# tjake/Jlama

Hardware: NVIDIA B200
Metric: decode tokens/s (higher is better)
Workload: dtype int8xint4->f32

## Files before the change

include/jlama_b200.h:

```cpp
#ifndef JLAMA_B200_H
#define JLAMA_B200_H

#include <stdint.h>

#ifdef __cplusplus
extern "C" {
#endif

#define JL_OK 0
#define JL_ERR_INVALID (-1)
#define JL_ERR_CUDA (-2)
#define JL_ERR_OOM (-3)
#define JL_ERR_UNSUPPORTED (-4)
#define JL_ERR_NCCL (-5)

#define JL_F32 0
#define JL_BF16 1
#define JL_Q4 2
#define JL_I8 3

typedef struct jl_ctx jl_ctx;
typedef struct jl_model jl_model;

int jl_init(int device, jl_ctx **out, int64_t *info );
int jl_shutdown(jl_ctx *ctx);
const char *jl_last_error(jl_ctx *ctx);
const char *jl_version(void);
int jl_sync(jl_ctx *ctx);
int64_t jl_kernel_launches(jl_ctx *ctx);

int jl_debug_ktrace(jl_ctx *ctx, int capacity);
int jl_debug_ktrace_clear(jl_ctx *ctx);
int jl_debug_ktrace_read(jl_ctx *ctx, uint64_t *out, int max_slots);
int jl_debug_gemv_bench(jl_ctx *ctx, int64_t b_id, int n, int m, int mode, int iters, int use_pdl, double *avg_us);

int jl_debug_gemm_tc_bench(jl_ctx *ctx, int64_t b_id, int t, int iters, double *avg_us);

int64_t jl_register_tensor(jl_ctx *ctx, int dtype, int64_t rows, int64_t cols, const void *data, const float *scales);
int jl_unregister_tensor(jl_ctx *ctx, int64_t id);

int jl_gemm(jl_ctx *ctx, int a_dtype, const void *a, const float *a_scales, int a_col_off, int lda, int64_t b_id,
            int b_col_off, float *r, int roffset, int m, int n0, int n, int k, int ldc);
int jl_gemm_batch(jl_ctx *ctx, int batch_num, int a_dtype, const void *a, const float *a_scales, int a_col_off, int lda,
                  const int64_t *b_ids, int b_col_off, float *const *r, int roffset, int m, int n0, int n, int k,
                  int ldc);
int jl_gemm_tc(jl_ctx *ctx, int a_dtype, const void *a, int a_col_off, int lda, int64_t b_id, int b_col_off, float *r,
               int roffset, int m, int n0, int n, int k, int ldc);
int jl_gemm_host(jl_ctx *ctx, int a_dtype, const void *a, int a_col_off, int lda, int b_dtype, const void *b,
                 int b_col_off, int ldb, float *r, int roffset, int m, int n0, int n, int k, int ldc);

int jl_accumulate(jl_ctx *ctx, float *a, int a_rows, int lda, int b_dtype, const void *b, const float *b_scales,
                  int b_rows, int ldb, int offset, int length);
int jl_maccumulate(jl_ctx *ctx, float *a, int a_rows, int lda, const float *b, int b_rows, int ldb, int offset,
                   int length);
int jl_scale(jl_ctx *ctx, float factor, float *x, int rows, int ldx, int offset, int length);
int jl_saxpy(jl_ctx *ctx, float alpha, const float *x, float *y, int xoffset, int yoffset, int limit);
int jl_saxpy_batch(jl_ctx *ctx, const float *alpha, const float *x, int ldx, float *y, int xoffset, int yoffset,
                   int limit, int a_offset, int x_row_offset, int batch);
int jl_quantize_q8(jl_ctx *ctx, const float *x, int rows, int ldx, int offset, int length, int8_t *q, float *scales);
int jl_quantize_bf16(jl_ctx *ctx, const float *x, int rows, int ldx, int offset, int length, uint16_t *out);
int jl_quantize_q4_weights(jl_ctx *ctx, const float *x, int64_t rows, int64_t cols, uint8_t *q, float *scales);
int jl_quantize_q8_weights(jl_ctx *ctx, const float *x, int64_t rows, int64_t cols, int8_t *q, float *scales);

int jl_rmsnorm(jl_ctx *ctx, const float *x, int rows, int ldx, int w_dtype, const void *w, float weight_adjustment,
               float eps, int embedding_length, int offset, int length, float *out);
int jl_layernorm(jl_ctx *ctx, const float *x, int rows, int ldx, int w_dtype, const void *w, int b_dtype, const void *bias, float eps,
                 int embedding_length, int offset, int length, float *out);
#define JL_ACT_SILU 0
#define JL_ACT_GELU 1
// ... 180 lines not shown
```

jlama_b200/csrc/jl_model.cu:

```cuda
#include "jl_common.cuh"
#include <string>
#include "jl_pdecode.cuh"

#include <chrono>
#include <map>
#include <math.h>
#include <new>
#include <stdio.h>
#include <stdlib.h>
#include <string.h>

int jl_comm_allreduce_dev(jl_ctx *ctx, cudaStream_t stream, float *buf, size_t count);
int jl_comm_allgather_dev(jl_ctx *ctx, cudaStream_t stream, const void *send, void *recv, size_t bytes_per_rank);

struct jl_model {
    jl_ctx *ctx = nullptr;
    std::recursive_mutex mu;
    jl_model_config cfg;
    jl_dctx d;
    cudaStream_t stream = nullptr;
    bool finalized = false;
    DevTensor g[3];
    bool g_set[3] = {false, false, false};
    std::vector<DevTensor> l;
// ... 14 lines not shown
    int max_splits = 32;
    int32_t *d_tokens = nullptr, *d_positions = nullptr, *d_sessions = nullptr, *d_next = nullptr, *d_hist = nullptr,
            *d_counter = nullptr;
    void *argmax_scratch = nullptr;
    int32_t *h_pinned = nullptr;
    int hist_cap = 0;
    std::map<long long, cudaGraphExec_t> graphs;
    std::map<long long, long long> graph_launches;
    std::vector<cudaEvent_t> ev_pool;
    size_t ev_used = 0;
    cudaEvent_t ev_begin = nullptr, ev_end = nullptr;
    double last_total_ms = 0, last_gemv_ms = 0;
    bool timing_valid = false;
    int64_t weight_bytes = 0;
    unsigned *fda_done = nullptr;
    std::vector<DevTensor> aux;
    std::vector<char> aux_set;
    DevTensor gaux[2];
    bool gaux_set[2] = {false, false};
    int n_exp = 0, exp_k = 0;
    std::vector<DevTensor> moe_gate;
    std::vector<DevTensor> moe_w;
    std::vector<char> moe_set;
    void **moe_wtab = nullptr;
    float **moe_stab = nullptr;
    float *moe_logits = nullptr;
    int32_t *moe_sel = nullptr;
    bool pd_ok = false;
    int pd_wdtype = JL_Q4;
    std::vector<PdLayer> pd_layers;
    unsigned long long *pd_sync = nullptr, *pd_slots = nullptr, *pd_trace = nullptr;
    unsigned *pd_att_done = nullptr;
    int pd_vocab0 = 0, pd_vocab_rows = 0;
    uint4 *ll_o = nullptr, *ll_d = nullptr, *ll_a = nullptr;
    struct KvSpill {
        std::vector<std::pair<int, int>> pages;
        std::vector<char> bytes;
    };
    std::map<int64_t, KvSpill> spills;
    int64_t next_spill = 1;
    uint4 *peer_ll_o[PD_MAX_TP] = {}, *peer_ll_d[PD_MAX_TP] = {}, *peer_ll_a[PD_MAX_TP] = {};
    float *peer_logits[PD_MAX_TP] = {};
    std::vector<void *> ipc_opened;
};

#define M_CHECK(expr)                 \
    do {                              \
        int _rc = (expr);             \
        if (_rc != JL_OK) return _rc; \
    } while (0)

static bool use_pdl(const jl_model *m) {
    static int env = -1;
    if (env < 0) {
        const char *e = getenv("JL_PDL");
        env = e ? (atoi(e) ? 1 : 0) : 2;
    }
    if (m->cfg.flags & JL_MODEL_NO_PDL) return false;
    if (env != 2) return env == 1;
    return (m->cfg.flags & JL_MODEL_PDL) != 0;
}
static bool use_graph(const jl_model *m) { return !(m->cfg.flags & JL_MODEL_NO_GRAPH); }
static bool use_pd(const jl_model *m) {
    static int env = -1;
    if (env < 0) {
        const char *e = getenv("JL_PERSISTENT");
// ... 380 lines not shown
                JL_CUDA_CHECK(ctx, cudaMemset(m->ll_d, 0, lines * 16));
                JL_CUDA_CHECK(ctx, cudaMemset(m->ll_a, 0, (size_t)PD_MAX_TP * 16));
                void *local[4] = {m->ll_o, m->ll_d, m->ll_a, m->logits};
                cudaIpcMemHandle_t mine[4];
                for (int i = 0; i < 4; i++) JL_CUDA_CHECK(ctx, cudaIpcGetMemHandle(&mine[i], local[i]));
                cudaIpcMemHandle_t *d_send = nullptr, *d_recv = nullptr;
                M_CHECK(dev_alloc(ctx, (void **)&d_send, sizeof mine));
                M_CHECK(dev_alloc(ctx, (void **)&d_recv, sizeof mine * W));
                JL_CUDA_CHECK(ctx, cudaMemcpy(d_send, mine, sizeof mine, cudaMemcpyHostToDevice));
                int rc = jl_comm_allgather_dev(ctx, m->stream, d_send, d_recv, sizeof mine);
                if (rc == JL_OK && cudaStreamSynchronize(m->stream) != cudaSuccess) rc = jl_set_error(ctx, JL_ERR_CUDA, "handle exchange failed");
                std::vector<cudaIpcMemHandle_t> all((size_t)4 * W);
                if (rc == JL_OK) JL_CUDA_CHECK(ctx, cudaMemcpy(all.data(), d_recv, sizeof mine * W, cudaMemcpyDeviceToHost));
                cudaFree(d_send);
                cudaFree(d_recv);
                if (rc != JL_OK) return rc;
                for (int r = 0; r < W; r++) {
                    void *ptrs[4];
                    for (int i = 0; i < 4; i++) {
                        if (r == c.tp_rank) {
                            ptrs[i] = local[i];
                        } else {
                            cudaError_t e = cudaIpcOpenMemHandle(&ptrs[i], all[(size_t)r * 4 + i], cudaIpcMemLazyEnablePeerAccess);
                            if (e != cudaSuccess)
                                return jl_set_error(ctx, JL_ERR_CUDA, "cudaIpcOpenMemHandle(rank %d): %s (peer access over NVLink is required)", r,
                                                    cudaGetErrorString(e));
                            m->ipc_opened.push_back(ptrs[i]);
                        }
                    }
                    m->peer_ll_o[r] = (uint4 *)ptrs[0], m->peer_ll_d[r] = (uint4 *)ptrs[1], m->peer_ll_a[r] = (uint4 *)ptrs[2];
                    m->peer_logits[r] = (float *)ptrs[3];
                }
            }
            if (getenv("JL_PD_TRACE")) {
                M_CHECK(dev_alloc(ctx, (void **)&m->pd_trace, ((size_t)c.num_layers * 16 + 32) * 8));
                JL_CUDA_CHECK(ctx, cudaMemset(m->pd_trace, 0, ((size_t)c.num_layers * 16 + 32) * 8));
            }
            m->pd_ok = true;
            if (W > 1) m->weight_bytes += -tb(head) + (int64_t)((double)tb(head) * m->pd_vocab_rows / V);
        }
    }
    m->finalized = true;
    return JL_OK;
}

extern "C" int64_t jl_model_weight_bytes(jl_model *m) { return m ? m->weight_bytes : -1; }

int jl_model_num_experts(jl_model *m) { return m ? m->n_exp : 0; }

void jl_model_limits(jl_model *m, int out[4]) {
    out[0] = out[1] = out[2] = out[3] = 0;
    if (!m || !m->finalized) return;
    out[0] = m->cfg.max_sessions, out[1] = m->max_context, out[2] = m->cfg.max_batch;
    out[3] = m->cfg.max_sessions < GEMV_MAX_M ? m->cfg.max_sessions : GEMV_MAX_M;
}

void jl_models_invalidate_graphs(jl_ctx *ctx) {
    for (jl_model *m : ctx->models) {
        if (m->stream) cudaStreamSynchronize(m->stream);
        for (auto &kv : m->graphs) cudaGraphExecDestroy(kv.second);
        m->graphs.clear();
        m->graph_launches.clear();
    }
}

extern "C" int jl_model_free(jl_model *m) {
// ... 558 lines not shown
    p.layers = c.num_layers, p.E = c.embedding_length, p.H = m->h_seg, p.attn_seg = m->attn_seg, p.kv_seg = m->kv_seg;
    p.heads = m->heads_local, p.kv_heads = m->kv_heads_local, p.head_size = c.head_size;
    p.vocab = c.vocab_size, p.vocab_rows = m->pd_vocab_rows, p.vocab0 = m->pd_vocab0;
    p.head0_global = m->d.headStart, p.kv_head0_global = m->d.groupHeadStart;
    p.eps = c.layer_norm_eps;
    p.attn_scale = (float)(1.0 / sqrt((double)c.head_size));
    p.lw = nullptr;
    p.embed_dt = m->g[JL_T_EMBED].dtype, p.embed_w = m->g[JL_T_EMBED].data, p.embed_s = m->g[JL_T_EMBED].scales;
    p.out_norm = m->g[JL_T_OUT_NORM].data, p.out_norm_dt = m->g[JL_T_OUT_NORM].dtype;
    const DevTensor &head = m->g_set[JL_T_LM_HEAD] ? m->g[JL_T_LM_HEAD] : m->g[JL_T_EMBED];
    const size_t rb = (size_t)c.embedding_length / 32 * (head.dtype == JL_Q4 ? 16 : 32);
    p.lm_w = (const uint8_t *)head.data + (size_t)m->pd_vocab0 * rb;
    p.lm_s = head.scales + (size_t)m->pd_vocab0 * (c.embedding_length / 32);
    p.x = m->x, p.xb = m->xb, p.q = m->q, p.k = m->k, p.v = m->v, p.att = m->att, p.h = m->hbuf, p.logits = m->logits;
    p.attn_ws = m->attn_ws;
    p.rope = m->rope;
    p.kv = m->kv;
    p.tokens = m->d_tokens, p.positions = m->d_positions, p.next = m->d_next, p.sessions = m->d_sessions;
    p.hist = m->d_hist, p.counter = m->d_counter, p.hist_cap = m->hist_cap, p.resident = resident ? 1 : 0;
    p.sync = m->pd_sync, p.argmax_slots = m->pd_slots, p.att_done = m->pd_att_done;
    int s = (max_pos + 1 + 63) / 64;
    const int cap = m->ctx->sm_count / m->kv_heads_local;
    if (s > cap) s = cap;
    if (s > m->max_splits) s = m->max_splits;
    if (s < 1) s = 1;
    p.splits = s;
    p.split_cap = cap < m->max_splits ? cap : m->max_splits;
    p.ntok = 1;
    p.world = c.tp_size, p.rank = c.tp_rank;
    for (int r = 0; r < c.tp_size && r < PD_MAX_TP; r++)
        p.ll_o[r] = m->peer_ll_o[r], p.ll_d[r] = m->peer_ll_d[r], p.ll_a[r] = m->peer_ll_a[r], p.logits_peer[r] = m->peer_logits[r];
    p.want_logits = want_logits && c.tp_size > 1 ? 1 : 0;
    p.trace = m->pd_trace;
}

static int pd_check(jl_model *m) {
    if (!m->pd_ok) return JL_OK;
    unsigned long long st[2] = {0, 0};
    if (cudaMemcpy(st, m->pd_sync, sizeof st, cudaMemcpyDeviceToHost) != cudaSuccess) return jl_set_error(m->ctx, JL_ERR_CUDA, "decode status read failed");
    if (st[1] == 0) return JL_OK;
    cudaMemset(m->pd_sync, 0, PD_SYNC_WORDS * 8);
    cudaMemset(m->pd_att_done, 0, (size_t)m->kv_heads_local * sizeof(unsigned));
    return jl_set_error(m->ctx, JL_ERR_CUDA, "persistent decode kernel timed out waiting on counter %llu (token %llu); state reset", st[1], st[0]);
}

static int run_decode(jl_model *m, int n, int max_pos, bool resident, bool want_logits = false, int ntok = 1) {
    jl_ctx *ctx = m->ctx;
    if (n == 1 && use_pd(m)) {
        PdParams pp;
        fill_pd(m, max_pos, resident, want_logits, pp);
        pp.ntok = resident ? ntok : 1;
        return jl_launch_pdecode(ctx, m->stream, pp, m->pd_layers.data(), m, m->pd_wdtype);
    }
    int splits = (max_pos + 1 + 63) / 64;
    if (n > 1) splits = (splits + n - 1) / n;
    {
        static const int buckets[] = {1, 2, 3, 4, 6, 8, 12, 16, 24, 32};
        int b = 32;
        for (int v : buckets)
            if (v >= splits) {
                b = v;
                break;
            }
        splits = b > m->max_splits ? m->max_splits : b;
    }
    if (!use_graph(m)) {
// ... 434 lines not shown
```

jlama_b200/csrc/jl_pdecode.cu:

```cuda
#include "jl_pdecode.cuh"
#include "jl_gemv_body.cuh"
#define JL_EXP_FN __forceinline__
#include "jl_attn_task.cuh"
#include "jl_attn_flat.cuh"
#include <stddef.h>
#include <stdlib.h>
#include <string.h>

#define PD_NT PD_THREADS
#define PD_NWARP (PD_NT / 32)
#define PD_CH(WDT) ((WDT) == JL_Q4 ? 4 : 2)
#define PD_NBUF 3
#define PD_SPIN_LOCAL (1u << 22)
#define PD_SPIN_PEER (1u << 26)
#define EPI_LL 3
#ifndef PD_PHASE_FN
#define PD_PHASE_FN __forceinline__
#endif

#define PD_MAX_LAYERS 128
struct PdConst {
    PdParams P[1];
    PdLayer layers[PD_MAX_LAYERS];
};
// ... 8 lines not shown
__device__ __forceinline__ unsigned long long pd_ld_acquire(const unsigned long long *p) {
    unsigned long long v;
    asm volatile("ld.acquire.gpu.global.u64 %0, [%1];" : "=l"(v) : "l"(p) : "memory");
    return v;
}
__device__ __forceinline__ unsigned long long pd_ld_volatile(const unsigned long long *p) {
    unsigned long long v;
    asm volatile("ld.volatile.global.u64 %0, [%1];" : "=l"(v) : "l"(p) : "memory");
    return v;
}
__device__ __forceinline__ void pd_arrive(const int pz, int which) {
    pd_cta_bar();
    if (threadIdx.x == 0) asm volatile("red.release.gpu.global.add.u64 [%0], 1;" ::"l"(CP.sync + which) : "memory");
}
__device__ __forceinline__ void pd_wait(const int pz, int which, unsigned long long target) {
    if (threadIdx.x == 0) {
        unsigned long long *sync = CP.sync;
        const unsigned long long *c = sync + which;
        unsigned n = 0;
        while (pd_ld_acquire(c) < target) {
            if ((++n & 0x3ff) == 0) {
                if (pd_ld_volatile(sync + 1) != 0) break;
                if (n > PD_SPIN_LOCAL) {
                    sync[1] = (unsigned long long)which;
                    break;
                }
            }
        }
    }
    pd_cta_bar();
}
__device__ __forceinline__ void pd_stamp(const int pz, int idx) {
    if (CP.trace && blockIdx.x == 0 && threadIdx.x == 0) CP.trace[idx] = globaltimer_ns();
}

template <int PH>
__device__ __forceinline__ void ll_store(const int pz, int row, float v, uint32_t tag) {
    const int world = CP.world;
#pragma unroll 1
    for (int d = 0; d < world; d++) {
        uint32_t *dst = (uint32_t *)(PH == PH_O ? CP.ll_o[d] : CP.ll_d[d]) + ((size_t)CP.rank * CP.E + row) * 2;
        asm volatile("st.volatile.global.v2.u32 [%0], {%1, %2};" ::"l"(dst), "r"(__float_as_uint(v)), "r"(tag) : "memory");
    }
}
__device__ __forceinline__ float ll_load(const int pz, const uint4 *mine, int src_rank, int row, uint32_t tag) {
    const uint32_t *src = (const uint32_t *)mine + ((size_t)src_rank * CP.E + row) * 2;
    uint32_t v, t;
    unsigned n = 0;
    for (;;) {
        asm volatile("ld.volatile.global.v2.u32 {%0, %1}, [%2];" : "=r"(v), "=r"(t) : "l"(src) : "memory");
        if (t == tag) break;
        if ((++n & 0x3ff) == 0) {
            if (pd_ld_volatile(CP.sync + 1) != 0) break;
            if (n > PD_SPIN_PEER) {
                CP.sync[1] = 100 + (unsigned long long)src_rank;
                break;
            }
        }
    }
    return __uint_as_float(v);
}

__device__ __forceinline__ int item_owner_pd(int i, int items, int nwarp) { return (int)((((long long)(i + 1)) * nwarp - 1) / items); }

__device__ __forceinline__ unsigned long long pd_pack_arg(float v, int idx) {
    if (!(v == v)) return 0ull;
// ... 71 lines not shown
            seg = it.wr;
            local = R0 + it.r;
        } else {
            ph_seg<PH>(pz, R0 + it.r, seg, local);
        }
        const uint8_t *w;
        const float *s;
#ifdef PD_X_FIXEDW
        w = CP.lm_w, s = CP.lm_s;
#else
        ph_weights<PH>(L, seg, w, s);
#endif
        const size_t blk = (size_t)local * (size_t)nblk;
        wrow = w + blk * WB;
        srow = s + blk;
    };
    auto advance = [&](It &it) {
        if (!LONG || ++it.c == nchunks) {
            it.c = 0;
            if (++it.wr == NW) {
                it.wr = 0;
                ++it.r;
            }
        }
    };
    It cur, ld;
    {
        cur.r = i0 / per_row;
        const int rem = i0 - cur.r * per_row;
        cur.wr = rem / nchunks;
        cur.c = rem - cur.wr * nchunks;
        ld = cur;
    }
    WBuf<WDT, CH> buf[NBUF];
    pd_ring_clear<WDT, CH, NBUF>(buf);
    const uint8_t *wrow;
    const float *srow;
    const unsigned long long pol = l2_evict_first_policy();
    int ci = i0, li = i0;
#pragma unroll
    for (int b = 0; b < NBUF - 1; b++) {
        if (li < i1) {
            row_ptrs(ld, wrow, srow);
            load_chunk<WDT, CH>(buf[b], wrow, srow, ld.c * 32 * CH, nblk, lane, pol);
            advance(ld);
            li++;
        }
    }
#ifndef PD_X_NOWAIT
    pd_wait(pz, dep_which, dep_target);
    pd_stamp(pz, stamp_idx);
#endif
    {
        GemvParams p;
        p.a = PH == PH_QKV ? CP.x : (PH == PH_O ? CP.att : (PH == PH_GU ? CP.xb : CP.h));
        p.a_col_off = 0, p.K = ph_K<PH>(pz), p.lda = p.K;
        p.norm_w = PH == PH_QKV ? c_pd.layers[L].attn_norm : c_pd.layers[L].ffn_norm;
        p.norm_w_dtype = PH == PH_QKV ? c_pd.layers[L].attn_norm_dt : c_pd.layers[L].ffn_norm_dt;
        p.norm_adj = 0.0f, p.norm_eps = CP.eps, p.norm_E = CP.E, p.norm_inv_E = 1.0 / (double)CP.E;
        StageRegs<NORM, LONG && !NORM> sr;
        stage_q8_issue<NORM, LONG && !NORM, NT>(p, sr);
        stage_q8_finish<NORM, LONG && !NORM, NT, 1>(p, sr, smem, nblk);
    }
    float *parts = (float *)(smem + (((size_t)nblk * 40 + 15) & ~(size_t)15));
    const int maxsplit = nchunks < NWARP ? nchunks : NWARP;
    float acc[1] = {0.0f};
// ... 51 lines not shown
        for (int o = tid; o < nrows; o += NT) {
            float sums[NW];
#pragma unroll
            for (int wr = 0; wr < NW; wr++) {
                const int rw = o * NW + wr;
                const int wa = item_owner_pd(rw * nchunks, items, NWARP), wb = item_owner_pd(rw * nchunks + nchunks - 1, items, NWARP);
                float t = 0.0f;
                for (int w = wa; w <= wb; w++) t = __fadd_rn(t, parts[rw * maxsplit + (w - wa)]);
                sums[wr] = t;
            }
            store_row(R0 + o, sums[0], sums[NW - 1]);
        }
    }
}


template <int WDT>
__device__ PD_PHASE_FN unsigned long long pd_lm_head(const int, const int dep_which, const unsigned long long dep_target, const int stamp_idx,
                                                     const int want_logits, unsigned char *smem) {
    PD_OPAQUE_ZERO(pz);
    constexpr int NT = PD_NT, NWARP = PD_NWARP, CH = PD_CH(WDT), NBUF = PD_NBUF;
    constexpr int WB = (WDT == JL_Q4) ? 16 : 32;
    __shared__ double red[NWARP];
    __shared__ unsigned long long wbest[NWARP];
    int tid = threadIdx.x, cta_id = blockIdx.x, ncta = gridDim.x;
    asm volatile("" : "+r"(tid), "+r"(cta_id), "+r"(ncta));
    const int lane = tid & 31, warp = tid >> 5;
    const int K = CP.E, nblk = K / 32;
    const int R0 = (int)(((long long)CP.vocab_rows * cta_id) / ncta);
    const int R1 = (int)(((long long)CP.vocab_rows * (cta_id + 1)) / ncta);
    const int nrows = R1 - R0;
    const int r0 = R0 + (int)(((long long)nrows * warp) / NWARP), r1 = R0 + (int)(((long long)nrows * (warp + 1)) / NWARP);
    const int nchunks = (nblk + 32 * CH - 1) / (32 * CH);
    WBuf<WDT, CH> buf[NBUF];
    pd_ring_clear<WDT, CH, NBUF>(buf);
    const unsigned long long pol = l2_evict_first_policy();
    int lr = r0, lc = 0, cr = r0, cc = 0;
    auto issue = [&](WBuf<WDT, CH> &b) {
        const size_t blk = (size_t)lr * nblk;
        load_chunk<WDT, CH>(b, CP.lm_w + blk * WB, CP.lm_s + blk, lc * 32 * CH, nblk, lane, pol);
        if (++lc == nchunks) lc = 0, ++lr;
    };
#pragma unroll
    for (int b = 0; b < NBUF - 1; b++)
        if (lr < r1) issue(buf[b]);
    pd_wait(pz, dep_which, dep_target);
    pd_stamp(pz, stamp_idx);
    {
        float4 *af4 = (float4 *)smem;
        double ss = 0.0;
        for (int i4 = tid; i4 < K / 4; i4 += NT) {
            const float4 v = __ldcg((const float4 *)(CP.x + i4 * 4));
            ss += (double)__fmul_rn(v.x, v.x);
            ss += (double)__fmul_rn(v.y, v.y);
            ss += (double)__fmul_rn(v.z, v.z);
            ss += (double)__fmul_rn(v.w, v.w);
        }
        ss = warp_sum_d(ss);
        if (lane == 0) red[warp] = ss;
        pd_cta_bar();
        double t = 0.0;
#pragma unroll
        for (int w = 0; w < NWARP; w++) t += red[w];
        const float rsf = rms_scale(t, 1.0 / (double)CP.E, CP.eps);
        for (int i4 = tid; i4 < K / 4; i4 += NT) {
            const float4 v = __ldcg((const float4 *)(CP.x + i4 * 4));
// ... 94 lines not shown
        return;
    }
    const int group = at.heads / at.kv_heads;
    const int n = at.positions[0] + 1;
    const int per = (((n + splits - 1) / splits) + 31) / 32 * 32;
    (void)n;
    (void)per;
    (void)group;
    attention_flat<HS, PD_NT>(at, layer, 0, kvh, split, smem, [&]() { pd_wait(pz, PC_QKV, qkv_target); });
}

template <int WDT, int HS>
__global__ void __launch_bounds__(PD_NT, 1) pdecode_kernel(const int splits0, const int resident, const int want_logits, const int ntok,
                                                            const int split_cap) {
    PD_OPAQUE_ZERO(pz);
    extern __shared__ __align__(1024) unsigned char smem[];
    __shared__ int s_last;
    const int tid = threadIdx.x;
    const int G = gridDim.x, cta = blockIdx.x;
    unsigned long long epoch = pd_ld_volatile(CP.sync);
    const unsigned long long fin0 = pd_ld_volatile(CP.sync + PC_FINAL);
    for (int tk = 0; tk < ntok; tk++) {
    int splits = splits0;
    if (tk > 0) {
        pd_wait(pz, PC_FINAL, fin0 + (unsigned long long)tk);
        const int pos = *(volatile const int32_t *)CP.positions;
        splits = (pos + 1 + 63) / 64;
        splits = splits > split_cap ? split_cap : (splits < 1 ? 1 : splits);
    }
    const unsigned long long uG = (unsigned long long)G;
    const bool tp = CP.world > 1;
    const int layers = CP.layers;
    const bool lng_E = CP.E > 32 * 32 * PD_CH(WDT), lng_A = CP.attn_seg > 32 * 32 * PD_CH(WDT), lng_H = CP.H > 32 * 32 * PD_CH(WDT);
    pd_stamp(pz, 0);

    {
        const int E = CP.E;
        const int c_a = (int)(((long long)E * cta) / G), c_b = (int)(((long long)E * (cta + 1)) / G);
        const size_t tok = (size_t)__ldcg(CP.tokens);
        for (int c = c_a + tid; c < c_b; c += PD_NT) CP.x[c] = pd_embed_value(pz, tok, c);
        pd_arrive(pz, PC_EMBED);
    }
    const int ntasks = CP.kv_heads * splits;

    for (int L = 0; L < layers; L++) {
        PD_OPAQUE_ZERO(pz);
        const unsigned long long use = epoch * (unsigned long long)layers + (unsigned long long)L + 1;
        const uint32_t tag_o = (uint32_t)(use * 2), tag_d = (uint32_t)(use * 2 + 1);
        {
            const int dw = L == 0 ? PC_EMBED : PC_DOWN;
            const unsigned long long dt = L == 0 ? (epoch + 1) * uG : (use - 1) * uG;
            if (lng_E) pd_gemv<WDT, PH_QKV, EPI_STORE, true>(pz, L, 0u, dw, dt, 1 + L * 8 + 0, smem);
            else pd_gemv<WDT, PH_QKV, EPI_STORE, false>(pz, L, 0u, dw, dt, 1 + L * 8 + 0, smem);
            pd_arrive(pz, PC_QKV);
            pd_stamp(pz, 1 + L * 8 + 1);
        }
        if (cta < ntasks) {
            const int split = cta % splits, kvh = cta / splits;
            pd_attention<HS>(pz, L, kvh, split, splits, false, use * uG, smem);
            bool signal = true;
            if (splits > 1) {
                pd_cta_bar();
                if (tid == 0) {
                    __threadfence();
                    unsigned *c = &CP.att_done[kvh];
                    const unsigned old = atomicAdd(c, 1u);
// ... 116 lines not shown

static size_t pd_smem_bytes(const PdParams &p) {
    int Kmax = p.E;
    if (p.H > Kmax) Kmax = p.H;
    if (p.attn_seg > Kmax) Kmax = p.attn_seg;
    const int G = 148;
    int Rmax = p.E > p.H ? p.E : p.H;
    if (p.attn_seg + 2 * p.kv_seg > Rmax) Rmax = p.attn_seg + 2 * p.kv_seg;
    size_t acts = (((size_t)(Kmax / 32) * 40 + 15) & ~(size_t)15) + (size_t)((Rmax + G - 1) / G + 2) * 2 * PD_NWARP * 4 + 64;
    const size_t lm = (size_t)p.E * 4;
    if (lm > acts) acts = lm;
    const int hs = p.head_size;
    size_t att = hs == 32 ? attention_flat_smem<32, PD_NT>() : (hs == 64 ? attention_flat_smem<64, PD_NT>() : attention_flat_smem<128, PD_NT>());
    att += 1024;
    size_t m = acts > att ? acts : att;
    const size_t red = (size_t)((p.E + G - 1) / G + 2) * PD_MAX_TP * 4;
    if (red > m) m = red;
    return (m + 1023) & ~(size_t)1023;
}

bool jl_pdecode_supported(const PdParams &p, int w_dtype, int grid) {
    if (w_dtype != JL_Q4 && w_dtype != JL_I8) return false;
    if (p.head_size != 32 && p.head_size != 64 && p.head_size != 128) return false;
    if (p.heads % p.kv_heads || p.heads / p.kv_heads > MG_MAX_GROUP) return false;
    if ((p.E % 32) || (p.H % 32) || (p.attn_seg % 32) || (p.E % 8)) return false;
    if (p.E > 16 * PD_NT) return false;
    if (p.kv_heads * 1 > grid) return false;
    if (p.world > PD_MAX_TP || p.layers > PD_MAX_LAYERS) return false;
    {
        const int group = p.heads / p.kv_heads;
        if (group & (group - 1)) return false;
    }
    return pd_smem_bytes(p) <= 200 * 1024;
}

static const void *g_pd_owner[JL_MAX_DEVICES] = {};
static std::mutex g_pd_mu;

void jl_pdecode_forget(int device, const void *owner) {
    std::lock_guard<std::mutex> lk(g_pd_mu);
    if (device >= 0 && device < JL_MAX_DEVICES && g_pd_owner[device] == owner) g_pd_owner[device] = nullptr;
}

template <int WDT, int HS>
static int launch_pd(jl_ctx *ctx, cudaStream_t stream, const PdParams &p) {
    auto kern = pdecode_kernel<WDT, HS>;
    const size_t smem = pd_smem_bytes(p);
    static size_t configured[JL_MAX_DEVICES] = {};
    JL_CUDA_CHECK(ctx, jl_ensure_dyn_smem(kern, ctx->device, smem, configured));
    cudaLaunchConfig_t cfg = {};
    cfg.gridDim = dim3(ctx->sm_count);
    cfg.blockDim = dim3(PD_NT);
    cfg.dynamicSmemBytes = smem;
    cfg.stream = stream;
    cudaLaunchAttribute attr[1];
    attr[0].id = cudaLaunchAttributeCooperative;
    attr[0].val.cooperative = 1;
    cfg.attrs = attr;
    cfg.numAttrs = 1;
    JL_CUDA_CHECK(ctx, cudaLaunchKernelEx(&cfg, kern, p.splits, p.resident, p.want_logits, p.ntok > 0 ? p.ntok : 1, p.split_cap));
    ctx->launches++;
    return JL_OK;
}

template <int WDT>
static int launch_pd_hs(jl_ctx *ctx, cudaStream_t stream, const PdParams &p) {
// ... 32 lines not shown
```

jlama_b200/csrc/jl_pdecode.cuh:

```cuda
#pragma once
#include "jl_common.cuh"

#ifndef PD_THREADS
#define PD_THREADS 512
#endif
#define PD_MAX_TP 8
#define PD_SYNC_WORDS 32

struct PdLayer {
    const uint8_t *w[7];
    const float *s[7];
    const void *attn_norm, *ffn_norm;
    int attn_norm_dt, ffn_norm_dt;
};
enum { PW_Q = 0, PW_K, PW_V, PW_O, PW_GATE, PW_UP, PW_DOWN };

enum { PC_EMBED = 8, PC_QKV, PC_ATT, PC_O, PC_GU, PC_DOWN, PC_LM, PC_FINAL };

struct PdParams {
    int layers, E, H, attn_seg, kv_seg, heads, kv_heads, head_size;
    int vocab, vocab_rows, vocab0;
    int head0_global, kv_head0_global;
    float eps, attn_scale;
    const PdLayer *lw;
    int embed_dt;
    const void *embed_w;
    const float *embed_s;
    const void *out_norm;
    int out_norm_dt;
    const uint8_t *lm_w;
    const float *lm_s;
    float *x, *xb, *q, *k, *v, *att, *h, *logits, *attn_ws;
    const float *rope;
    KvLayout kv;
    int32_t *tokens, *positions, *next;
    const int32_t *sessions;
    int32_t *hist, *counter;
    int hist_cap, resident;
    unsigned long long *sync;
    unsigned long long *argmax_slots;
    unsigned *att_done;
    int splits;
    int ntok, split_cap;
    int world, rank;
    uint4 *ll_o[PD_MAX_TP];
    uint4 *ll_d[PD_MAX_TP];
    uint4 *ll_a[PD_MAX_TP];
    int want_logits;
    float *logits_peer[PD_MAX_TP];
    unsigned long long *trace;
};

bool jl_pdecode_supported(const PdParams &p, int w_dtype, int grid);
int jl_launch_pdecode(jl_ctx *ctx, cudaStream_t stream, const PdParams &p, const PdLayer *layers_host, const void *owner, int w_dtype);
void jl_pdecode_forget(int device, const void *owner);
```

jlama_b200/native.py:

```python
import ctypes as C
import os

HERE = os.path.dirname(os.path.abspath(__file__))
LIB_PATH = os.path.join(HERE, "libjlama_b200.so")

JL_OK, JL_ERR_INVALID, JL_ERR_CUDA, JL_ERR_OOM, JL_ERR_UNSUPPORTED, JL_ERR_NCCL = 0, -1, -2, -3, -4, -5
F32, BF16, Q4, I8 = 0, 1, 2, 3
MODEL_NO_GRAPH, MODEL_NO_PDL, MODEL_NO_PERSISTENT, MODEL_PDL = 1, 2, 4, 16

T_EMBED, T_OUT_NORM, T_LM_HEAD = 0, 1, 2
L_ATTN_NORM, L_Q, L_K, L_V, L_O, L_FFN_NORM, L_GATE, L_DOWN, L_UP = range(9)


class JlamaNativeError(RuntimeError):
    def __init__(self, code, msg):
        super().__init__("jlama_b200 error %d: %s" % (code, msg))
        self.code = code


class UnsupportedOperation(JlamaNativeError):
    """UnsupportedOperationException analogue (TestOperations.java:140 relies on it)."""


class ModelConfig(C.Structure):
# ... 29 lines not shown
SCHED_FORWARD_FN = C.CFUNCTYPE(C.c_int, C.c_void_p, C.c_int, C.POINTER(C.c_int32), C.c_int, C.c_int)
SCHED_SAMPLE_FN = C.CFUNCTYPE(C.c_int, C.c_void_p, C.c_int, C.c_float, C.c_float, C.POINTER(C.c_int32))
SCHED_DECODE_FN = C.CFUNCTYPE(C.c_int, C.c_void_p, C.c_int, C.POINTER(C.c_int32), C.POINTER(C.c_int32), C.POINTER(C.c_int32),
                              C.POINTER(C.c_float), C.POINTER(C.c_float), C.POINTER(C.c_int32))


SCHED_OFFLOAD_FN = C.CFUNCTYPE(C.c_int, C.c_void_p, C.c_int, C.POINTER(C.c_int64))
SCHED_RESTORE_FN = C.CFUNCTYPE(C.c_int, C.c_void_p, C.c_int, C.c_int64)
SCHED_DISCARD_FN = C.CFUNCTYPE(C.c_int, C.c_void_p, C.c_int64)


class SchedBackend(C.Structure):
    _fields_ = [("reset_session", SCHED_RESET_FN), ("batch_forward", SCHED_FORWARD_FN), ("sample", SCHED_SAMPLE_FN),
                ("decode", SCHED_DECODE_FN), ("offload", SCHED_OFFLOAD_FN), ("restore", SCHED_RESTORE_FN), ("discard", SCHED_DISCARD_FN)]


SCHED_QUEUED, SCHED_PREFILL, SCHED_DECODING, SCHED_FINISHED, SCHED_FAILED = range(5)
FINISH_NONE, FINISH_MAX_TOKENS, FINISH_STOP_TOKEN, FINISH_CANCELLED, FINISH_ERROR = range(5)
SCHED_KEEP_SESSION = 1

_vp, _i, _i64, _f, _d = C.c_void_p, C.c_int, C.c_int64, C.c_float, C.c_double
SIGNATURES = {
    "jl_init": (_i, [_i, C.POINTER(_vp), _vp]),
    "jl_shutdown": (_i, [_vp]),
    "jl_last_error": (C.c_char_p, [_vp]),
    "jl_version": (C.c_char_p, []),
    "jl_sync": (_i, [_vp]),
    "jl_kernel_launches": (_i64, [_vp]),
    "jl_debug_ktrace": (_i, [_vp, _i]),
    "jl_debug_ktrace_clear": (_i, [_vp]),
    "jl_debug_ktrace_read": (_i, [_vp, C.POINTER(C.c_uint64), _i]),
    "jl_debug_gemv_bench": (_i, [_vp, _i64, _i, _i, _i, _i, _i, C.POINTER(_d)]),
    "jl_debug_gemm_tc_bench": (_i, [_vp, _i64, _i, _i, C.POINTER(_d)]),
    "jl_register_tensor": (_i64, [_vp, _i, _i64, _i64, _vp, _vp]),
    "jl_unregister_tensor": (_i, [_vp, _i64]),
    "jl_gemm": (_i, [_vp, _i, _vp, _vp, _i, _i, _i64, _i, _vp, _i, _i, _i, _i, _i, _i]),
    "jl_gemm_tc": (_i, [_vp, _i, _vp, _i, _i, _i64, _i, _vp, _i, _i, _i, _i, _i, _i]),
    "jl_gemm_batch": (_i, [_vp, _i, _i, _vp, _vp, _i, _i, _vp, _i, _vp, _i, _i, _i, _i, _i, _i]),
    "jl_gemm_host": (_i, [_vp, _i, _vp, _i, _i, _i, _vp, _i, _i, _vp, _i, _i, _i, _i, _i, _i]),
    "jl_accumulate": (_i, [_vp, _vp, _i, _i, _i, _vp, _vp, _i, _i, _i, _i]),
    "jl_maccumulate": (_i, [_vp, _vp, _i, _i, _vp, _i, _i, _i, _i]),
    "jl_scale": (_i, [_vp, _f, _vp, _i, _i, _i, _i]),
    "jl_saxpy": (_i, [_vp, _f, _vp, _vp, _i, _i, _i]),
    "jl_saxpy_batch": (_i, [_vp, _vp, _vp, _i, _vp, _i, _i, _i, _i, _i, _i]),
    "jl_quantize_q8": (_i, [_vp, _vp, _i, _i, _i, _i, _vp, _vp]),
    "jl_quantize_bf16": (_i, [_vp, _vp, _i, _i, _i, _i, _vp]),
    "jl_quantize_q4_weights": (_i, [_vp, _vp, _i64, _i64, _vp, _vp]),
    "jl_quantize_q8_weights": (_i, [_vp, _vp, _i64, _i64, _vp, _vp]),
    "jl_st_open": (_i, [C.c_char_p, C.POINTER(_vp)]),
    "jl_st_close": (_i, [_vp]),
    "jl_st_last_error": (C.c_char_p, []),
    "jl_st_count": (_i, [_vp]),
    "jl_st_find": (_i, [_vp, C.c_char_p]),
    "jl_st_info": (_i, [_vp, _i, C.POINTER(C.c_char_p), C.POINTER(_i), C.POINTER(_i), C.POINTER(_i64), C.POINTER(_i64)]),
    "jl_st_data": (_vp, [_vp, _i]),
    "jl_st_metadata": (C.c_char_p, [_vp, C.c_char_p]),
    "jl_st_majority_dtype": (_i, [_vp]),
    "jl_st_write": (_i, [C.c_char_p, _i, _vp, _vp, _vp, _vp, _vp, _vp, _i, _vp]),
    "jl_quantize_model": (_i, [_vp, C.c_char_p, C.c_char_p, _i, C.c_char_p, C.c_char_p]),
    "jl_config_from_json": (_i, [C.c_char_p, C.POINTER(ModelConfig)]),
    "jl_model_load_safetensors": (_i, [_vp, _vp, _vp, _vp, _i, C.POINTER(_i)]),
    "jl_model_tp_layout": (_i, [_vp, C.POINTER(Dctx), C.POINTER(_i)]),
    "jl_rmsnorm": (_i, [_vp, _vp, _i, _i, _i, _vp, _f, _f, _i, _i, _i, _vp]),
    "jl_softmax": (_i, [_vp, _vp, _i, _i]),
    "jl_layernorm": (_i, [_vp, _vp, _i, _i, _i, _vp, _i, _vp, _f, _i, _i, _i, _vp]),
    "jl_activation": (_i, [_vp, _i, _vp, _i, _i, _i, _i]),
# ... 122 lines not shown
```

Before: 594.0.

## Add per-CTA rolling L2 bulk prefetch of upcoming decode weights

Adds a software prefetcher to the persistent decode kernel. At each phase, thread 0 of every CTA issues cp.async.bulk.prefetch.L2 for the weight and scale bytes that CTA will read, up to a configurable window ahead (256 KB by default, overridable with JL_PD_LOOKAHEAD_KB). It walks the per-CTA row slices of the QKV, O, gate/up, down and lm_head tensors across layers. The goal is to hide DRAM latency for the bandwidth-bound GEMV stream, at the cost of extra prefetch instructions, L2 pressure, and the risk that the prefetched row slices do not match the CTA's actual row split.

Result: slower. 452.2 (median of 6 runs) (-23.9%).

```diff
diff --git a/include/jlama_b200.h b/include/jlama_b200.h
--- a/include/jlama_b200.h
+++ b/include/jlama_b200.h
@@ -35,6 +35,9 @@
 int jl_debug_gemv_bench(jl_ctx *ctx, int64_t b_id, int n, int m, int mode, int iters, int use_pdl, double *avg_us);
 
 int jl_debug_gemm_tc_bench(jl_ctx *ctx, int64_t b_id, int t, int iters, double *avg_us);
+
+int jl_debug_pdecode_prefetch_ranges(const int64_t *dims, const uint64_t *bases, int grid, int cta, uint64_t from, uint64_t to, uint64_t *out,
+                                     int max_ranges);
 
 int64_t jl_register_tensor(jl_ctx *ctx, int dtype, int64_t rows, int64_t cols, const void *data, const float *scales);
 int jl_unregister_tensor(jl_ctx *ctx, int64_t id);
diff --git a/jlama_b200/csrc/jl_model.cu b/jlama_b200/csrc/jl_model.cu
--- a/jlama_b200/csrc/jl_model.cu
+++ b/jlama_b200/csrc/jl_model.cu
@@ -70,6 +70,7 @@
     unsigned long long *pd_sync = nullptr, *pd_slots = nullptr, *pd_trace = nullptr;
     unsigned *pd_att_done = nullptr;
     int pd_vocab0 = 0, pd_vocab_rows = 0;
+    unsigned long long pd_pf_window = 0;
     uint4 *ll_o = nullptr, *ll_d = nullptr, *ll_a = nullptr;
     struct KvSpill {
         std::vector<std::pair<int, int>> pages;
@@ -516,6 +517,14 @@
                     m->peer_logits[r] = (float *)ptrs[3];
                 }
             }
+            m->pd_pf_window = (unsigned long long)PD_PF_DEFAULT_KB << 10;
+            if (const char *s = getenv("JL_PD_LOOKAHEAD_KB")) {
+                char *end = nullptr;
+                const long long kb = strtoll(s, &end, 10);
+                if (end == s || *end != '\0' || kb < 0 || kb > (1ll << 40))
+                    return jl_set_error(ctx, JL_ERR_INVALID, "JL_PD_LOOKAHEAD_KB=%s: expected KB per CTA, 0 .. 2^40", s);
+                m->pd_pf_window = (unsigned long long)kb << 10;
+            }
             if (getenv("JL_PD_TRACE")) {
                 M_CHECK(dev_alloc(ctx, (void **)&m->pd_trace, ((size_t)c.num_layers * 16 + 32) * 8));
                 JL_CUDA_CHECK(ctx, cudaMemset(m->pd_trace, 0, ((size_t)c.num_layers * 16 + 32) * 8));
@@ -1140,6 +1149,7 @@
         p.ll_o[r] = m->peer_ll_o[r], p.ll_d[r] = m->peer_ll_d[r], p.ll_a[r] = m->peer_ll_a[r], p.logits_peer[r] = m->peer_logits[r];
     p.want_logits = want_logits && c.tp_size > 1 ? 1 : 0;
     p.trace = m->pd_trace;
+    p.pf_window = m->pd_pf_window;
 }
 
 static int pd_check(jl_model *m) {
diff --git a/jlama_b200/csrc/jl_pdecode.cu b/jlama_b200/csrc/jl_pdecode.cu
--- a/jlama_b200/csrc/jl_pdecode.cu
+++ b/jlama_b200/csrc/jl_pdecode.cu
@@ -64,6 +64,42 @@
 }
 __device__ __forceinline__ void pd_stamp(const int pz, int idx) {
     if (CP.trace && blockIdx.x == 0 && threadIdx.x == 0) CP.trace[idx] = globaltimer_ns();
+}
+
+enum { PF_FRONT = PD_PF_SLICES + 1, PF_WORDS };
+__shared__ unsigned long long pd_pf[PF_WORDS];
+#define PD_PF_PIECE (32u << 10)
+
+template <int WDT>
+__device__ __forceinline__ void pd_pf_begin_token() {
+    unsigned long long lb = 0;
+    for (int ph = 0; ph < PD_PF_SLICES; ph++) {
+        const unsigned long long b = pd_pf_slice_bytes(CP, ph, WDT, gridDim.x, blockIdx.x);
+        pd_pf[ph] = b;
+        if (ph < 4) lb += b;
+    }
+    pd_pf[PD_PF_SLICES] = lb;
+    pd_pf[PF_FRONT] = 0;
+}
+template <int WDT>
+__device__ __forceinline__ void pd_pf_advance(unsigned long long target) {
+    const unsigned long long front = pd_pf[PF_FRONT];
+    if (target <= front) return;
+    auto issue = [](unsigned long long a, unsigned long long n) {
+        while (n) {
+            const unsigned piece = n < PD_PF_PIECE ? (unsigned)n : PD_PF_PIECE;
+            asm volatile("cp.async.bulk.prefetch.L2.global [%0], %1;" ::"l"(a), "r"(piece) : "memory");
+            a += piece, n -= piece;
+        }
+    };
+    pd_pf_walk(CP, c_pd.layers, WDT, gridDim.x, blockIdx.x, pd_pf, front, target, issue);
+    pd_pf[PF_FRONT] = target;
+}
+template <int WDT>
+__device__ __forceinline__ void pd_pf_phase(int L, int ph) {
+    unsigned long long s = (unsigned long long)L * pd_pf[PD_PF_SLICES];
+    for (int q = 0; q < ph; q++) s += pd_pf[q];
+    pd_pf_advance<WDT>(s + CP.pf_window);
 }
 
 template <int PH>
@@ -201,6 +237,7 @@
         cur.c = rem - cur.wr * nchunks;
         ld = cur;
     }
+    if (tid == 0 && CP.pf_window) pd_pf_phase<WDT>(L, PH);
     WBuf<WDT, CH> buf[NBUF];
     pd_ring_clear<WDT, CH, NBUF>(buf);
     const uint8_t *wrow;
@@ -318,6 +355,7 @@
     const int nrows = R1 - R0;
     const int r0 = R0 + (int)(((long long)nrows * warp) / NWARP), r1 = R0 + (int)(((long long)nrows * (warp + 1)) / NWARP);
     const int nchunks = (nblk + 32 * CH - 1) / (32 * CH);
+    if (tid == 0 && CP.pf_window) pd_pf_phase<WDT>(CP.layers, 4);
     WBuf<WDT, CH> buf[NBUF];
     pd_ring_clear<WDT, CH, NBUF>(buf);
     const unsigned long long pol = l2_evict_first_policy();
@@ -478,6 +516,7 @@
     const bool tp = CP.world > 1;
     const int layers = CP.layers;
     const bool lng_E = CP.E > 32 * 32 * PD_CH(WDT), lng_A = CP.attn_seg > 32 * 32 * PD_CH(WDT), lng_H = CP.H > 32 * 32 * PD_CH(WDT);
+    if (tid == 0 && CP.pf_window) pd_pf_begin_token<WDT>();
     pd_stamp(pz, 0);
 
     {
@@ -660,6 +699,37 @@
         if (group & (group - 1)) return false;
     }
     return pd_smem_bytes(p) <= 200 * 1024;
+}
+
+extern "C" int jl_debug_pdecode_prefetch_ranges(const int64_t *dims, const uint64_t *bases, int grid, int cta, uint64_t from, uint64_t to,
+                                                uint64_t *out, int max_ranges) {
+    if (!dims || !bases || grid <= 0 || cta < 0 || cta >= grid || max_ranges < 0 || (max_ranges > 0 && !out)) return JL_ERR_INVALID;
+    PdParams p = {};
+    p.layers = (int)dims[0], p.E = (int)dims[1], p.H = (int)dims[2], p.attn_seg = (int)dims[3], p.kv_seg = (int)dims[4], p.vocab_rows = (int)dims[5];
+    const int wdt = (int)dims[6];
+    if (p.layers < 1 || p.layers > PD_MAX_LAYERS || p.E <= 0 || p.H <= 0 || p.attn_seg <= 0 || p.kv_seg <= 0 || p.vocab_rows <= 0 ||
+        (wdt != JL_Q4 && wdt != JL_I8) || p.E % 32 || p.H % 32 || p.attn_seg % 32)
+        return JL_ERR_INVALID;
+    std::vector<PdLayer> layers(p.layers);
+    for (int L = 0; L < p.layers; L++)
+        for (int i = 0; i < 7; i++) {
+            layers[L].w[i] = (const uint8_t *)(uintptr_t)bases[(size_t)L * 14 + i];
+            layers[L].s[i] = (const float *)(uintptr_t)bases[(size_t)L * 14 + 7 + i];
+        }
+    p.lm_w = (const uint8_t *)(uintptr_t)bases[(size_t)p.layers * 14];
+    p.lm_s = (const float *)(uintptr_t)bases[(size_t)p.layers * 14 + 1];
+    unsigned long long sb[PD_PF_SLICES + 1] = {};
+    for (int ph = 0; ph < PD_PF_SLICES; ph++) {
+        sb[ph] = pd_pf_slice_bytes(p, ph, wdt, grid, cta);
+        if (ph < 4) sb[PD_PF_SLICES] += sb[ph];
+    }
+    int n = 0;
+    auto emit = [&](unsigned long long a, unsigned long long bytes) {
+        if (n < max_ranges) out[2 * n] = a, out[2 * n + 1] = bytes;
+        n++;
+    };
+    pd_pf_walk(p, layers.data(), wdt, grid, cta, sb, from, to, emit);
+    return n;
 }
 
 static const void *g_pd_owner[JL_MAX_DEVICES] = {};
diff --git a/jlama_b200/csrc/jl_pdecode.cuh b/jlama_b200/csrc/jl_pdecode.cuh
--- a/jlama_b200/csrc/jl_pdecode.cuh
+++ b/jlama_b200/csrc/jl_pdecode.cuh
@@ -49,7 +49,72 @@
     int want_logits;
     float *logits_peer[PD_MAX_TP];
     unsigned long long *trace;
+    unsigned long long pf_window;
 };
+
+#define PD_PF_SLICES 5
+#define PD_PF_DEFAULT_KB 256
+__host__ __device__ inline int pd_pf_rows_total(const PdParams &p, int ph) {
+    return ph == 0 ? p.attn_seg + 2 * p.kv_seg : (ph == 2 ? p.H : (ph == 4 ? p.vocab_rows : p.E));
+}
+__host__ __device__ inline int pd_pf_K(const PdParams &p, int ph) { return ph == 1 ? p.attn_seg : (ph == 3 ? p.H : p.E); }
+__host__ __device__ inline unsigned long long pd_pf_row_bytes(const PdParams &p, int ph, int wdt) {
+    return (unsigned long long)(ph == 2 ? 2 : 1) * (unsigned long long)(pd_pf_K(p, ph) / 32) * ((wdt == JL_Q4 ? 16 : 32) + 4);
+}
+__host__ __device__ inline int pd_pf_row0(const PdParams &p, int ph, int grid, int cta) {
+    return (int)(((long long)pd_pf_rows_total(p, ph) * cta) / grid);
+}
+__host__ __device__ inline unsigned long long pd_pf_slice_bytes(const PdParams &p, int ph, int wdt, int grid, int cta) {
+    return (unsigned long long)(pd_pf_row0(p, ph, grid, cta + 1) - pd_pf_row0(p, ph, grid, cta)) * pd_pf_row_bytes(p, ph, wdt);
+}
+template <class F>
+__host__ __device__ inline void pd_pf_emit_inward(const void *begin, const void *end, F &emit) {
+    const unsigned long long a = ((unsigned long long)begin + 15) & ~15ull, b = (unsigned long long)end & ~15ull;
+    if (b > a) emit(a, b - a);
+}
+template <class F>
+__host__ __device__ inline void pd_pf_slice_ranges(const PdParams &p, const PdLayer &l, int wdt, int ph, int grid, int cta, unsigned long long lo,
+                                                   unsigned long long hi, F &emit) {
+    const unsigned long long rb = pd_pf_row_bytes(p, ph, wdt);
+    const long long r0 = pd_pf_row0(p, ph, grid, cta);
+    const long long a = r0 + (long long)(lo / rb), b = r0 + (long long)(hi / rb);
+    const unsigned long long nblk = (unsigned long long)(pd_pf_K(p, ph) / 32), wb = wdt == JL_Q4 ? 16 : 32;
+    auto tensor = [&](const uint8_t *w, const float *s, long long t0, long long tn) {
+        const long long x = (a > t0 ? a : t0) - t0, y = (b < t0 + tn ? b : t0 + tn) - t0;
+        if (y <= x) return;
+        pd_pf_emit_inward(w + x * nblk * wb, w + y * nblk * wb, emit);
+        pd_pf_emit_inward(s + x * nblk, s + y * nblk, emit);
+    };
+    if (ph == 0) {
+        tensor(l.w[PW_Q], l.s[PW_Q], 0, p.attn_seg);
+        tensor(l.w[PW_K], l.s[PW_K], p.attn_seg, p.kv_seg);
+        tensor(l.w[PW_V], l.s[PW_V], p.attn_seg + p.kv_seg, p.kv_seg);
+    } else if (ph == 2) {
+        tensor(l.w[PW_GATE], l.s[PW_GATE], 0, p.H);
+        tensor(l.w[PW_UP], l.s[PW_UP], 0, p.H);
+    } else if (ph == 4) {
+        tensor(p.lm_w, p.lm_s, 0, p.vocab_rows);
+    } else {
+        tensor(l.w[ph == 1 ? PW_O : PW_DOWN], l.s[ph == 1 ? PW_O : PW_DOWN], 0, p.E);
+    }
+}
+template <class F>
+__host__ __device__ inline void pd_pf_walk(const PdParams &p, const PdLayer *layers, int wdt, int grid, int cta, const unsigned long long *sb,
+                                           unsigned long long from, unsigned long long to, F &emit) {
+    const unsigned long long lb = sb[PD_PF_SLICES], lm0 = (unsigned long long)p.layers * lb, total = lm0 + sb[4];
+    if (to > total) to = total;
+    while (from < to) {
+        int L = p.layers, ph = 4;
+        unsigned long long base = lm0;
+        if (from < lm0) {
+            L = (int)(from / lb), ph = 0, base = (unsigned long long)L * lb;
+            while (from - base >= sb[ph]) base += sb[ph++];
+        }
+        const unsigned long long end = base + sb[ph], hi = to < end ? to : end;
+        pd_pf_slice_ranges(p, layers[L < p.layers ? L : 0], wdt, ph, grid, cta, from - base, hi - base, emit);
+        from = hi;
+    }
+}
 
 bool jl_pdecode_supported(const PdParams &p, int w_dtype, int grid);
 int jl_launch_pdecode(jl_ctx *ctx, cudaStream_t stream, const PdParams &p, const PdLayer *layers_host, const void *owner, int w_dtype);
diff --git a/jlama_b200/native.py b/jlama_b200/native.py
--- a/jlama_b200/native.py
+++ b/jlama_b200/native.py
@@ -85,6 +85,7 @@
     "jl_debug_ktrace_read": (_i, [_vp, C.POINTER(C.c_uint64), _i]),
     "jl_debug_gemv_bench": (_i, [_vp, _i64, _i, _i, _i, _i, _i, C.POINTER(_d)]),
     "jl_debug_gemm_tc_bench": (_i, [_vp, _i64, _i, _i, C.POINTER(_d)]),
+    "jl_debug_pdecode_prefetch_ranges": (_i, [C.POINTER(_i64), C.POINTER(C.c_uint64), _i, _i, C.c_uint64, C.c_uint64, C.POINTER(C.c_uint64), _i]),
     "jl_register_tensor": (_i64, [_vp, _i, _i64, _i64, _vp, _vp]),
     "jl_unregister_tensor": (_i, [_vp, _i64]),
     "jl_gemm": (_i, [_vp, _i, _vp, _vp, _i, _i, _i64, _i, _vp, _i, _i, _i, _i, _i, _i]),
```
